# luigifcruz/radio-core

Measured on AMD Instinct MI355X. Metric: IQ Msamples/s through Tuner+WBFM at 1024 channels, higher is better.
Workload: dtype f32

## Files before the change

### include/rcfm_tools.h

```cpp
#ifndef RCFM_TOOLS_H
#define RCFM_TOOLS_H

#include "rcfm.h"

#ifdef __cplusplus
extern "C" {
#endif

typedef struct rcfm_arena_s* rcfm_arena_t;

int rcfm_arena_create(size_t block_bytes, rcfm_arena_t* out);
int rcfm_arena_adopt(void* base, size_t bytes, rcfm_arena_t* out);
int rcfm_arena_bind(rcfm_arena_t arena);
int rcfm_arena_stats(rcfm_arena_t arena, size_t* reserved_bytes, size_t* used_bytes, size_t* live_pieces);
int rcfm_arena_destroy(rcfm_arena_t arena);


enum { RCFM_TUNER_OPT_NARROW_TILES = 1,
       RCFM_TUNER_OPT_ALIGNED_PLAN = 2 };
int rcfm_tuner_set_option(rcfm_tuner_t t, int option, int value);
int rcfm_tuner_load_route(rcfm_tuner_t t, int format, int* route);

enum { RCFM_OPT_LDS_CHAIN = 1, RCFM_OPT_FUSED_TILES = 2, RCFM_OPT_PHASE_LINK = 3, RCFM_OPT_PILOT_CHAIN = 6, RCFM_OPT_DECIM_TILE = 7,
       RCFM_OPT_LDS_DEEMPH = 8, RCFM_OPT_PILOT_BLOCKED = 9, RCFM_OPT_SSB_DIRECT = 11 };
int rcfm_demod_get_option(rcfm_demod_t d, int option, int* value);


typedef struct rcfm_fft_pass {
    int32_t L, nstages, radix[8];
    int64_t n_o1, n_o2, n_inner;
    int64_t in_o1, in_o2, in_i, in_l;
    int64_t out_o1, out_o2, out_i, out_k;
    int64_t tw_o1, tw_o2, tw_i;
    int32_t has_twiddle, load_along_l;
    int64_t in_t, out_t;
    int32_t flat_outer;
    int32_t reserved_;
} rcfm_fft_pass;
typedef struct rcfm_fft_plan {
// ... 29 lines not shown
```

### radio-core_amd/csrc/demod.hip

```cpp

#include <cmath>
#include <cstring>

#include "agc.h"
#include "api_internal.h"

using namespace rcfm;

struct rcfm_demod_s {
    Arena* arena = arena_enter_handle();
    ~rcfm_demod_s() {
        drop_graphs();
        if (cap_stream) (void)hipStreamDestroy(cap_stream);
        arena_leave_handle(arena);
    }
    int kind = 0, C = 0, B = 0, A = 0, ch = 1, chunk = 1;
    double tau = 75e-6;
    float taps_h[51];
    float zi_h[50];
    float pilot_h[41];
    float pilot_g_h[41];
    DeviceBuffer taps, pilot_g;
    struct StateBuf : DeviceBuffer {
        hipEvent_t ev = nullptr;
// ... 18 lines not shown
    float* state_at(int first) const { return state_ptr() + (size_t)first * state_stride(); }
    float side_tap = 0.23f;
    ResampleGeom geom;
    PlanCache r2c_B, c2c_inv_B, c2c_fwd_B, c2c_inv_A, c2r_A;
    std::unique_ptr<FftEngine> eng_B, eng_A;
    std::unique_ptr<FftEngine> eng_Ad;
    std::unique_ptr<FftEngine> eng_Bi;
    DeviceBuffer buf_Ti;
    bool opt_lds_chain = true;
    bool opt_pilot_chain = true;
    bool opt_decim_tile = true;
    bool opt_pilot_blocked = true;
    bool opt_phase_link = true;
    bool opt_lds_deemph = true;
    bool opt_ssb_direct = true;
    int opt_narrow = kNarrowDefault;
    bool opt_graph = false;
    struct GraphSlot {
        const void* iq;
        void* audio;
        const float* state;
        int first;
        hipGraphExec_t exec;
        uint64_t used;
    };
    std::vector<GraphSlot> graphs;
    GraphSlot last_call{nullptr, nullptr, nullptr, -1, nullptr, 0};
    hipStream_t cap_stream = nullptr;
    uint64_t graph_tick = 0;
    void drop_graphs() {
        for (auto& g : graphs) (void)hipGraphExecDestroy(g.exec);
        graphs.clear();
        last_call = GraphSlot{nullptr, nullptr, nullptr, -1, nullptr, 0};
    }
    bool narrow(int cnt) const { return eng_B && narrow_launch(*eng_B, cnt, opt_narrow); }
    DeviceBuffer work, buf_iq, buf_m, buf_p, buf_P, buf_Z, buf_V, buf_v, partial, buf_T, buf_TA, buf_U2, buf_dc;
    int tiles = 0;

    bool decim_plan(const FftEngine& eb, int64_t fa[2]) const {
        const int64_t n1 = eb.desc().pass[0].L;
        fa[0] = A / n1;
        fa[1] = n1;
        FftPlanDesc pa;
        return A % (2 * n1) == 0 && A / n1 >= 16 && fft_plan_describe(A, &pa, 0, fa, 2);
    }

    bool stateful() const { return kind == RCFM_MFM || kind == RCFM_WBFM; }
    bool ssb() const { return kind == RCFM_USB || kind == RCFM_LSB; }

    bool agc_on = false;
    double agc_decay = 0.0;
// ... 68 lines not shown
            if (eng_B->desc().npass == 2 && A < B && decim_plan(*eng_B, fa)) {
                eng_Ad = std::make_unique<FftEngine>(A, fa, 2);
                buf_TA.reserve(c * eng_Ad->tmp_stride() * sizeof(float2));
                if (const int pitch = audio_pitch())
                    buf_V.reserve(c * (size_t)(A / eng_Ad->row_length()) * pitch * sizeof(float2));
            }
            if (kind != RCFM_WBFM) {
                buf_Z.reset(c * B * sizeof(float2));
                buf_V.reset(c * A * sizeof(float2));
            }
        }
        if (kind == RCFM_WBFM) {
            const size_t per_channel = std::max<size_t>((size_t)B, (size_t)pilot_blocked().stride);
            buf_m.reset(c * per_channel * sizeof(float));
            buf_p.reset(c * per_channel * sizeof(float));
        }
    }

    void reset_state(hipStream_t s) {
        if (agc_on) {
            const std::vector<float> all((size_t)C, -1.f);
            RC_HIP(hipMemcpyAsync(state_ptr(), all.data(), all.size() * sizeof(float), hipMemcpyHostToDevice, s));
            RC_HIP(hipStreamSynchronize(s));
        }
        if (!stateful()) return;
        std::vector<float> all((size_t)C * ch * 50);
        for (size_t i = 0; i < all.size(); ++i) all[i] = zi_h[i % 50];
        RC_HIP(hipMemcpyAsync(state_ptr(), all.data(), all.size() * sizeof(float), hipMemcpyHostToDevice, s));
        RC_HIP(hipStreamSynchronize(s));
    }
// ... 222 lines not shown
                TILE_CALL(nw, fused_pilot_chain_mask_mix, *eng_B, *eng_Bi, p, m, T, buf_Ti.as<float2>(), cnt, s, blk.stride,
                          blk.blk16());
            }
            paired = true;
        } else {
            {
                StageTimer tm(ST_FFT_REAL_B, s);
                TILE_CALL(nw, fused_real_pair_fft, *eng_B, p, U2, T, cnt, packed ? kKeepLowerHalf : -1, s);
            }
            if (eng_Bi && opt_pilot_chain) {
                StageTimer tm(ST_IFFT_B, s);
                paired = !packed ? TILE_CALL(nw, fused_hilbert_pair_ifft_mix_fft, *eng_Bi, *eng_B, U2, m, buf_Ti.as<float2>(), T, cnt, s)
                                 : TILE_CALL(nw, fused_hilbert_packed_ifft_mix_fft, *eng_Bi, *eng_B, U2, p, m,
                                             buf_Ti.as<float2>(), T, cnt, s);
            }
        }
        if (paired && eng_Ad && opt_decim_tile && TILE_CALL(nw, fused_fft_decim_ifft_applies, *eng_B, *eng_Ad, cnt)) {
            const int pitch = audio_pitch();
            {
                StageTimer tm(ST_FFT_B, s);
                TILE_CALL(nw, fused_fft_decim_ifft, *eng_B, *eng_Ad, T, V, TA, cnt, geom.wr.as<float>(), geom.scale,
                          buf_dc.as<float2>(), s, pitch);
            }
            run_deemph(reinterpret_cast<float*>(V), audio, first, cnt, s, false, pitch ? (int)eng_Ad->row_length() : 0, pitch);
            return;
        }
        if (paired) {
            StageTimer tm(ST_FFT_B, s);
            TILE_CALL(nw, fused_fft_last_pruned, *eng_B, T, Z, cnt, std::min(A, B) / 2, s);
        } else {
// ... 300 lines not shown

int rcfm_demod_set_option(rcfm_demod_t d, int option, int value) {
    return guarded([&] {
        RC_REQUIRE(d, RCFM_ERR_ARG, "NULL handle");
        d->drop_graphs();
        switch (option) {
            case RCFM_OPT_GRAPH: d->opt_graph = value != 0; break;
            case RCFM_OPT_LDS_CHAIN: d->opt_lds_chain = value != 0; break;
            case RCFM_OPT_FUSED_TILES: d->opt_pilot_chain = d->opt_decim_tile = value != 0; break;
            case RCFM_OPT_PILOT_CHAIN: d->opt_pilot_chain = value != 0; break;
            case RCFM_OPT_DECIM_TILE: d->opt_decim_tile = value != 0; break;
            case RCFM_OPT_PILOT_BLOCKED: d->opt_pilot_blocked = value != 0; break;
            case RCFM_OPT_LDS_DEEMPH: d->opt_lds_deemph = value != 0; break;
            case RCFM_OPT_PHASE_LINK: d->opt_phase_link = value != 0; break;
            case RCFM_OPT_SSB_DIRECT: d->opt_ssb_direct = value != 0; break;
            case RCFM_OPT_NARROW_TILES:
                RC_REQUIRE(value >= 0 && value <= 2, RCFM_ERR_ARG, "narrow tiles: 0 never, 1 automatic, 2 always");
                d->opt_narrow = value;
                break;
            case RCFM_OPT_STATE_FENCE: {
                auto& b = *d->state_buf;
                if (value != 0 && b.ev == nullptr) RC_HIP(hipEventCreateWithFlags(&b.ev, hipEventDisableTiming));
                b.armed = value != 0;
                if (!b.armed) b.recorded = false;
                break;
            }
            default: RC_REQUIRE(false, RCFM_ERR_ARG, "unknown demodulator option");
        }
    });
}
// ... 1 lines not shown
int rcfm_demod_get_option(rcfm_demod_t d, int option, int* value) {
    return guarded([&] {
        RC_REQUIRE(d && value, RCFM_ERR_ARG, "NULL handle or output");
        switch (option) {
            case RCFM_OPT_LDS_CHAIN: *value = d->opt_lds_chain; break;
            case RCFM_OPT_FUSED_TILES: *value = d->opt_pilot_chain && d->opt_decim_tile; break;
            case RCFM_OPT_PILOT_CHAIN: *value = d->opt_pilot_chain; break;
            case RCFM_OPT_DECIM_TILE: *value = d->opt_decim_tile; break;
            case RCFM_OPT_PILOT_BLOCKED:
                *value = d->opt_pilot_blocked && d->opt_pilot_chain && d->pilot_blocked().valid() &&
                         fused_pilot_chain_applies(*d->eng_B, *d->eng_Bi, 2);
                break;
            case RCFM_OPT_LDS_DEEMPH: *value = d->opt_lds_deemph; break;
            case RCFM_OPT_PHASE_LINK: *value = d->opt_phase_link; break;
            case RCFM_OPT_SSB_DIRECT: *value = d->opt_ssb_direct; break;
            case RCFM_OPT_NARROW_TILES: *value = d->opt_narrow; break;
            case RCFM_OPT_STATE_FENCE: *value = d->state_buf->armed; break;
            case RCFM_OPT_GRAPH: *value = d->opt_graph ? 1 + (int)d->graphs.size() : 0; break;
            default: RC_REQUIRE(false, RCFM_ERR_ARG, "unknown demodulator option");
        }
    });
}

int rcfm_demod_set_agc(rcfm_demod_t d, double decay_samples, float level, float floor) {
    return guarded([&] {
        RC_REQUIRE(d, RCFM_ERR_ARG, "NULL handle");
        RC_REQUIRE(d->kind == RCFM_AM || d->ssb(), RCFM_ERR_ARG, "AGC is for AM, USB and LSB demodulators");
        RC_REQUIRE(std::isfinite(decay_samples) && decay_samples >= 0.0, RCFM_ERR_ARG, "AGC decay_samples must be finite and >= 0");
        if (decay_samples == 0.0) {
            d->agc_on = false;
// ... 104 lines not shown
```

### radio-core_amd/csrc/fft_kernel.h

```cpp
#pragma once

#include <hip/hip_runtime.h>

#include <cstdio>
#include <cstdlib>
#include <type_traits>

#include "fft_engine.h"
#include "tile_ns.h"

namespace rcfm {
RCFM_NS_OPEN
namespace fftk {

constexpr int W = RCFM_TILE_W;
constexpr int kLogW = W == 16 ? 4 : W == 8 ? 3 : 2;
static_assert((1 << kLogW) == W, "tile width: 4, 8 or 16 lines");
constexpr int kThreads = 256 * W / 16;

__device__ __forceinline__ float2 cmul(float2 a, float2 b) {
    typedef float v2f __attribute__((ext_vector_type(2)));
    v2f A, B, D;
    A.x = a.x; A.y = a.y; B.x = b.x; B.y = b.y;
    asm("v_pk_mul_f32 %0, %1, %2 op_sel:[0,0] op_sel_hi:[0,1]" : "=v"(D) : "v"(A), "v"(B));
// ... 262 lines not shown
        return load.post(id, l, load.fetch(id, l, base, off), load.prepare(id));
    else
        return load.post(id, l, load.fetch(id, l, base, off));
}

template <class T, class = void>
struct has_half_zones : std::false_type {};
template <class T>
struct has_half_zones<T, std::void_t<decltype(T::kHalfZones)>> : std::bool_constant<T::kHalfZones> {};

template <class T, class = void>
struct has_aux : std::false_type {};
template <class T>
struct has_aux<T, std::void_t<decltype(T::kAux)>> : std::true_type {};

template <class StoreOp>
__device__ __forceinline__ void store_now(const StoreOp& store, const LineId& id, int k, int64_t base, unsigned off,
                                          float2 v) {
    if constexpr (has_aux<StoreOp>::value) store(id, k, base, off, v, store.fetch_aux(id, k, base, off));
    else store(id, k, base, off, v);
}

template <class LoadOp, class StoreOp>
__global__ __launch_bounds__(kThreads) void k_fft_pass(FftPassDev d, LoadOp load, StoreOp store) {
    extern __shared__ __attribute__((aligned(16))) unsigned char smem_raw[];
    const FftPass& p = d.p;
    const int L = p.L;
    float2* tile = reinterpret_cast<float2*>(smem_raw);
    float2* tw = tile + L * W;
    uint16_t* pos = reinterpret_cast<uint16_t*>(tw + L);

    const int tid = threadIdx.x;
    const int64_t tiles_inner = (p.n_inner + W - 1) / W;
    int64_t t = blockIdx.x;
// ... 345 lines not shown
    if constexpr (AUX) {
        const int wc = w < wvalid ? w : 0;
        id.i = i0 + wc;
#pragma unroll
        for (int it = 0; it < nitL; ++it) {
            int g = rg + RG * it;
            if (rowsL % RG != 0) g = g < rowsL ? g : 0;
            const int kb = kbase(g);
#pragma unroll
            for (int q = 0; q < RL; ++q) {
                const int k = kb + (L / RL) * q;
                aux[it * RL + q] = store.fetch_aux(id, k, out_base, (unsigned)k * out_k + (unsigned)wc);
            }
        }
    }

    if constexpr (ROWS) {
#pragma unroll
        for (int it = 0; it < nld; ++it) {
            const int e = tid + T * it;
            const int wl = e / L, l = e - wl * L;
            id.i = i0 + wl;
            float2 x;
            if constexpr (NF == 2) x = load.post(id, l, v[it], v2[it]);
            else x = load.post(id, l, v[it]);
            if ((L * W) % T == 0 || e < L * W) tile[lds_slot<true, !BIG>(l, wl)] = x;
        }
        __syncthreads();
        stage_lds<L, R0, L, true, RG, !BIG, BIG>(tile, tw, w, rg);
    } else {
// ... 57 lines not shown
            for (int q = 0; q < RL; ++q) x[q] = tile[lds_slot<ROWS, !BIG>(g * RL + q, w)];
            dft_p<RL>(x);
            const int kb = kbase(g);
            float2 Tw = make_float2(1.f, 0.f);
            if constexpr (PTW) Tw = big_twiddle(d, f * (unsigned)kb);
            if (lane_ok) {
#pragma unroll
                for (int q = 0; q < RL; ++q) {
                    const int k = kb + (L / RL) * q;
                    float2 y = x[dft_slot<RL>(q)];
                    if constexpr (PTW) {
                        y = cmul(y, Tw);
                        Tw = cmul(Tw, D);
                    }
                    if constexpr (AUX) store(id, k, out_base, (unsigned)k * out_k + (unsigned)w, y, aux[it * RL + q]);
                    else store(id, k, out_base, (unsigned)k * out_k + (unsigned)w, y);
                }
            }
        }
    }
}

template <class T, class = void>
struct mid_upper_rows_zero : std::false_type {};
template <class T>
struct mid_upper_rows_zero<T, std::void_t<decltype(T::kUpperRowsZero)>> : std::bool_constant<T::kUpperRowsZero> {};

template <int L, int R0, int R1, int R2, int R3, int T, class LoadOp, class MidOp, class StoreOp>
__global__ __launch_bounds__(T, (T * 16 / W >= 512 ? 4 : 1)) void k_fft_tile2(FftPassDev d1, FftPassDev d2, LoadOp load,
                                                                     MidOp mid, StoreOp store) {
// ... 560 lines not shown
                    win.dc_bin(id, x);
                }
                tile[lds_slot<true>(l, wl)] = make_float2(x.y, x.x);
            }
        }
        lds_barrier();

        stage_lds<L2, Q0, L2, true, RG>(tile, tw, w, rg);
        lds_barrier();
    }
    if constexpr (S2 == 3) {
        stage_lds<L2, Q1, L2 / Q0, true, RG>(tile, tw, w, rg);
        lds_barrier();
    }
    id.i = i0 + w;
    if (rg < rows2) {
        float2 x[QL];
#pragma unroll
        for (int q = 0; q < QL; ++q) x[q] = tile[lds_slot<true>(rg * QL + q, w)];
        dft_p<QL>(x);
        const float2 D = big_twiddle(d2, f * (unsigned)rows2, seedD);
        float2 Tw = big_twiddle(d2, f * (unsigned)kb2, seedT);
        if (w < wvalid) {
#pragma unroll
            for (int q = 0; q < QL; ++q) {
                const int k = kb2 + rows2 * q;
                const float2 y = cmul(x[dft_slot<QL>(q)], Tw);
                Tw = cmul(Tw, D);
                store(id, k, out_base, (unsigned)k * out_k + (unsigned)w, y);
            }
// ... 236 lines not shown
#define RCFM_CASE(LEN, A, B, C, D, LEN2, E, F, G) fast = fast || (d1.p.L == LEN && d2.p.L == LEN2);
    RCFM_FFT_DECIM_PAIRS(RCFM_CASE)
#undef RCFM_CASE
    return fast && d1.p.load_along_l && !d2.p.load_along_l &&
           d1.p.n_inner == d2.p.n_inner && d1.p.n_o1 * d1.p.n_o2 == 1 && d2.p.n_o1 * d2.p.n_o2 == 1 &&
           d1.p.out_k == d2.p.in_l && d2.p.in_i == 1 && d2.p.out_i == 1 && d2.p.has_twiddle && batch <= 65535;
}

template <class LoadOp, class WinOp, class StoreOp>
inline bool launch_fft_tile2_decim(const FftPassDev& d1, const FftPassDev& d2, int batch, const LoadOp& ld,
                                   const WinOp& win, const StoreOp& st, hipStream_t s) {
    if (!fft_tile2_decim_applies(d1, d2, batch)) return false;
    const dim3 grid((unsigned)((d1.p.n_inner + W - 1) / W), 1, (unsigned)batch);
    bool done = false;
#define RCFM_CASE(LEN, A, B, C, D, LEN2, E, F, G)                                                                \
    if (!done && d1.p.L == LEN && d2.p.L == LEN2) {                                                             \
        hipLaunchKernelGGL((k_fft_tile2_decim<LEN, A, B, C, D, LEN2, E, F, G, tile_threads(LEN), LoadOp, WinOp, StoreOp>), \
                           grid, dim3(tile_threads(LEN)), 0, s, d1, d2, ld, win, st);                           \
        done = true;                                                                                            \
    }
    RCFM_FFT_DECIM_PAIRS(RCFM_CASE)
#undef RCFM_CASE
    if (!done) return false;
    RC_HIP(hipGetLastError());
    return true;
}

template <class LoadOp, class MidOp, class StoreOp>
inline bool launch_fft_tile2_pair(const FftPassDev& d1, const FftPassDev& d2, int count, const LoadOp& ld,
                                  const MidOp& mid, const StoreOp& st, hipStream_t s) {
    const int pairs = (count + 1) / 2;
    if (!fft_tile2_applies(d1, d2, pairs)) return false;
    const dim3 grid((unsigned)((d1.p.n_inner + W - 1) / W), 1, (unsigned)pairs);
    switch (d1.p.L) {
// ... 36 lines not shown
```

### radio-core_amd/csrc/fused_passes.hip

```cpp
#include "fused_passes.h"
#include "device_math.h"

#include "fft_kernel.h"
#include "fft_decim_rt.h"
#include "kernels.h"

namespace rcfm {
RCFM_NS_OPEN

using fftk::LineId;
using fftk::kAnyPass;
using fftk::kRowsOnly;
using fftk::kStridedOnly;

namespace {


struct LoadTunerGatherFast {
    const float2* X;
    const int32_t* base;
    float two_pi_over_n, delta;
    float c0, c1, c2, c3;
    int B, nyq;
    int merge;
// ... 686 lines not shown
        const FftPassDev d1 = ef.pass_dev(1, ef.tmp_stride(), B), d2 = ea.pass_dev(0, A, ea.tmp_stride());
        RC_REQUIRE(fftk::launch_fft_tile2_decim(d1, d2, count, ld, win, st, s) || decim_rt(d1, d2, count, tmp_f, win, tmp_a, s),
                   RCFM_ERR_RUNTIME, "decimating two-transform kernel refused a pair it should accept");
    }
    fftk::LoadPlainT<false> ldl{tmp_a};
    fftk::StorePlainT<true> stl{out, 1.0f};
    FftPassDev last = ea.pass_dev(1, ea.tmp_stride(), A);
    if (out_pitch > 0) {
        RC_REQUIRE(out_pitch >= last.p.out_k && last.p.n_o1 * last.p.n_o2 == 1, RCFM_ERR_RUNTIME, "bad audio row pitch");
        last.out_batch = (A / last.p.out_k) * (int64_t)out_pitch;
        last.p.out_k = out_pitch;
    }
    fftk::launch_fft_pass<kRowsOnly>(last, count, ldl, stl, s);
}

struct StoreRealImagSplit {
    float* y;
    int n, count;
    __device__ __forceinline__ void operator()(const LineId& id, int, int64_t base, unsigned off, float2 v) const {
        const int64_t t = base + off - (int64_t)id.batch * n;
        const int c0 = 2 * id.batch;
        y[(int64_t)c0 * n + t] = v.y;
        if (c0 + 1 < count) y[(int64_t)(c0 + 1) * n + t] = v.x;
    }
};

void fused_real_pair_fft_first(const FftEngine& e, const float* x, float2* tmp, int count, bool from_phase,
                               hipStream_t s, PhaseRows rows) {
    if (count <= 0) return;
    const int64_t n = e.desc().n;
// ... 166 lines not shown
```

### radio-core_amd/csrc/fused_passes_decl.h

```cpp

namespace rcfm {
RCFM_DECL_NS_OPEN


void fused_tuner_ifft(const FftEngine& e, const TunerGather& g, float2* out, float2* tmp, int count,
                      hipStream_t s, float* theta = nullptr, int theta_pitch = 0, bool envelope = false);


void fused_real_fft(const FftEngine& e, const float* x, float2* U, float2* tmp, int count, int keep,
                    hipStream_t s);

void fused_hilbert_ifft(const FftEngine& e, const float2* U, float2* z, float2* tmp, int count, hipStream_t s);

void fused_real_pair_fft(const FftEngine& e, const float* x, float2* U2, float2* tmp, int count, int keep,
                         hipStream_t s, bool from_phase = false, PhaseRows rows = PhaseRows{});
void fused_hilbert_pair_ifft_mix(const FftEngine& e, const float2* U2, const float* m, float2* u, float2* tmp,
                                 int count, hipStream_t s);

bool fused_hilbert_pair_ifft_mix_fft(const FftEngine& ei, const FftEngine& ef, const float2* U2, const float* m,
                                     float2* tmp_i, float2* tmp_f, int count, hipStream_t s);
bool fused_hilbert_packed_applies(const FftEngine& ei, const FftEngine& ef, int count);
bool fused_hilbert_packed_ifft_mix_fft(const FftEngine& ei, const FftEngine& ef, const float2* U2, const float* p,
                                       const float* m, float2* tmp_i, float2* tmp_f, int count, hipStream_t s);
bool fused_pilot_chain_applies(const FftEngine& ef, const FftEngine& ei, int count);
bool fused_pilot_chain_geometry(const FftEngine& ef, int64_t* rows, int64_t* row_length);
void fused_pilot_chain_fft_first(const FftEngine& ef, const float* p, float2* tmp_f, int count, hipStream_t s,
                                 int64_t blk_stride = 0, int blk16 = 0);
void fused_pilot_chain_mask_mix(const FftEngine& ef, const FftEngine& ei, const float* p, const float* m,
                                float2* tmp_f, float2* tmp_i, int count, hipStream_t s, int64_t blk_stride = 0,
                                int blk16 = 0);

void fused_fft_last_pruned(const FftEngine& ef, const float2* tmp_f, float2* out, int count, int keep,
                           hipStream_t s);

bool fused_fft_decim_ifft_applies(const FftEngine& ef, const FftEngine& ea, int count);
void fused_fft_decim_ifft(const FftEngine& ef, const FftEngine& ea, const float2* tmp_f, float2* out, float2* tmp_a,
                          int count, const float* wr, float scale, float2* dc, hipStream_t s, int out_pitch = 0);

void fused_real_pair_fft_first(const FftEngine& e, const float* x, float2* tmp, int count, bool from_phase,
                               hipStream_t s, PhaseRows rows = PhaseRows{});
void fused_fft_decim_ifft_pairs(const FftEngine& ef, const FftEngine& ea, const float2* tmp_f, float* y,
                                float2* tmp_a, int count, const float* wr, float scale, float2* dc, hipStream_t s);

void fused_stereo_unpack_ifft(const FftEngine& e, const float2* U, int64_t B, float2* out, float2* tmp, int count,
                              const float* wr, int nyq, int nmin, float nyq_factor, float scale, float2* dc,
                              hipStream_t s);

void fused_fft_pruned(const FftEngine& e, const float2* in, float2* out, float2* tmp, int count, int keep,
                      hipStream_t s);

void fused_ifft_real_out(const FftEngine& e, const float2* Y, float* y, float2* tmp, int count, float scale,
                         hipStream_t s);

// ... 6 lines not shown
```

### radio-core_amd/csrc/kernels.h

```cpp
#pragma once

#include "common.h"

namespace rcfm {

enum NyquistMode : int { NYQ_NONE = 0, NYQ_DOWN = 1, NYQ_UP = 2 };

void launch_spectrum_c2c(const float2* X, int64_t x_stride, int64_t n, const int64_t* roll, float2* Y,
                         int64_t m, int batch, const float* wpos, const float* wneg, float w_merge,
                         int nyq, int nneg, int nyq_mode, float scale, hipStream_t stream);

void launch_spectrum_r2c(const float2* X, int64_t n, float2* Y, int64_t m, int batch, const float* wr,
                         int nyq, int nmin, float nyq_factor, float scale, hipStream_t stream);

void launch_spectrum_real_full(const float2* X, int64_t n, float2* Y, int64_t m, int batch, const float* wr,
                               int nyq, int nmin, float nyq_factor, float scale, float2* dc, bool paired,
                               hipStream_t stream);

void launch_hilbert_mask(const float2* P, float2* Z, int64_t n, int batch, float scale,
                         hipStream_t stream);

void launch_stereo_unpack(const float2* U, int64_t B, float2* V, int64_t A, int batch, const float* wr,
                          int nyq, int nmin, float nyq_factor, float scale, float2* dc, hipStream_t stream);

// ... 25 lines not shown

constexpr int kMaxBatch = 65535;
constexpr int kFirMaxTaps = 5461;
constexpr int kPilotMaxTaps = 2867;

int fir_tiles(int64_t n);
void launch_fir(const float* x, float* y, int64_t n, int ch, int batch, const float* taps, int nb,
                const float* state, float* partial, hipStream_t stream);
int fir51_tiles(int64_t n, int ch);
void launch_fir51(const float* x, float* y, int64_t n, int ch, int batch, const float* taps_host,
                  const float* state, float* partial, const float2* dc, hipStream_t stream, int row_samples = 0,
                  int row_pitch_samples = 0);
void launch_fir_state(const float* x, int64_t n, int ch, int batch, const float* taps, int nb,
                      float* state, hipStream_t stream, int row_samples = 0,
                      int row_pitch_samples = 0);
void launch_dc_clip(float* y, int64_t n, int ch, int batch, const float* partial, int nparts,
                    hipStream_t stream);

void launch_envelope(const float2* iq, float* e, int64_t n, hipStream_t stream);
void launch_am_tail(float* y, int64_t n, int batch, const float2* dc, hipStream_t stream);

void launch_ssb_select(const float2* X, int64_t n, float2* Y, int64_t m, int batch, const float* wr, int kmax,
                       int nyq_bin, float nyq_factor, float scale, bool lower, hipStream_t stream);
void launch_ssb_tail(float* y, int64_t n, int batch, float level, hipStream_t stream);

int level_segments(int64_t B);
void launch_channel_levels(const float2* X, int64_t N, const int32_t* base, const int64_t* roll, const int32_t* bw,
                           int count, int max_segments, double* part, float* power, hipStream_t stream);
struct CarrierPart {
    double s0, s1, s2, mx;
// ... 15 lines not shown
```

### radio-core_amd/csrc/kernels.hip

```cpp

#include "kernels.h"

#include <climits>
#include <cmath>
#include "device_math.h"

namespace rcfm {

namespace {

constexpr int kThreads = 256;
constexpr float kInvPi = 0.31830988618379067154f;

__device__ __forceinline__ float2 cscale(float2 a, float s) { return make_float2(a.x * s, a.y * s); }

inline dim3 grid2(int64_t items, int per_block, int batch) {
    return dim3((unsigned)((items + per_block - 1) / per_block), (unsigned)batch, 1);
}


__global__ __launch_bounds__(kThreads) void k_spectrum_c2c(
    const float2* __restrict__ X, int64_t x_stride, int64_t n, const int64_t* __restrict__ roll,
    float2* __restrict__ Y, int64_t m, const float* __restrict__ wpos, const float* __restrict__ wneg,
    float w_merge, int nyq, int nneg, int nyq_mode, float scale) {
// ... 680 lines not shown
    const int h = blockIdx.x % ch, c = blockIdx.x / ch;
    const float* xc = x + (int64_t)c * lay.signal_stride;
    float* zc = state + ((int64_t)c * ch + h) * (nb - 1);
    for (int s = threadIdx.x; s < nb - 1; s += blockDim.x) {
        z_old[s] = zc[s];
        xt[s] = (s < n) ? xc[lay.at((n - 1 - s) * ch + h)] : 0.f;
    }
    for (int s = threadIdx.x; s < nb; s += blockDim.x) tp[s] = taps[s];
    __syncthreads();
    for (int s = threadIdx.x; s < nb - 1; s += blockDim.x) {
        float acc = 0.f;
        const int cnt = (int)((nb - 1 - s) < n ? (nb - 1 - s) : n);
        for (int i = 0; i < cnt; ++i) acc = fmaf(tp[s + 1 + i], xt[i], acc);
        if (s + n < nb - 1) acc += z_old[s + n];
        zc[s] = acc;
    }
}

__global__ __launch_bounds__(kThreads) void k_dc_clip(float* __restrict__ y, int64_t total,
                                                      const float* __restrict__ partial, int nparts) {
    __shared__ float mean_s;
    const int c = blockIdx.y;
    if (threadIdx.x < 64) {
        double acc = 0.0;
        for (int i = threadIdx.x; i < nparts; i += 64) acc += (double)partial[(int64_t)c * nparts + i];
        for (int off = 32; off > 0; off >>= 1) acc += __shfl_down(acc, off, 64);
        if (threadIdx.x == 0) mean_s = (float)(acc / (double)total);
    }
    __syncthreads();
    const float mean = mean_s;
// ... 689 lines not shown
    if (ch == 2)
        hipLaunchKernelGGL(k_fir51<2>, grid, dim3(kThreads), 0, stream, x, y, n * 2, taps, state, partial, dc, lay);
    else
        hipLaunchKernelGGL(k_fir51<1>, grid, dim3(kThreads), 0, stream, x, y, n, taps, state, partial, dc, lay);
    RC_LAUNCH_CHECK();
}

void launch_fir_state(const float* x, int64_t n, int ch, int batch, const float* taps, int nb,
                      float* state, hipStream_t stream, int row_samples, int row_pitch_samples) {
    if (batch <= 0 || nb < 2) return;
    hipLaunchKernelGGL(k_fir_state, dim3((unsigned)(batch * ch)), dim3(128), fir_state_lds_bytes(nb), stream,
                       x, n, ch, taps, nb, state, row_layout(n, ch, row_samples, row_pitch_samples));
    RC_LAUNCH_CHECK();
}

void launch_dc_clip(float* y, int64_t n, int ch, int batch, const float* partial, int nparts,
                    hipStream_t stream) {
    if (batch <= 0) return;
    const int64_t total = n * ch;
    hipLaunchKernelGGL(k_dc_clip, grid2(total, kThreads, batch), dim3(kThreads), 0, stream, y, total, partial,
                       nparts);
    RC_LAUNCH_CHECK();
}

void launch_envelope(const float2* iq, float* e, int64_t n, hipStream_t stream) {
    if (n <= 0) return;
    if (((uintptr_t)iq | (uintptr_t)e) % 16 == 0)
        hipLaunchKernelGGL(k_envelope<true>, grid2((n + 3) / 4, kThreads, 1), dim3(kThreads), 0, stream, iq, e, n);
    else
        hipLaunchKernelGGL(k_envelope<false>, grid2(n, kThreads, 1), dim3(kThreads), 0, stream, iq, e, n);
// ... 128 lines not shown
```

### radio-core_amd/radiocore/_internal/hip.py

```python

import ctypes
import os
import sys
import threading
import warnings

import numpy as np

_HERE = os.path.dirname(os.path.abspath(__file__))
LIB_PATH = os.environ.get("RCFM_LIB") or os.path.join(os.path.dirname(_HERE), "_lib", "librcfm.so")

RCFM_FM, RCFM_MFM, RCFM_WBFM = 0, 1, 2
RCFM_AM = 3
RCFM_USB, RCFM_LSB = 5, 6
RCFM_SSB_LEVEL = 0.25
RCFM_AGC_PEAK, RCFM_AGC_CARRIER = 0, 1
RCFM_OPT_LDS_CHAIN, RCFM_OPT_FUSED_TILES, RCFM_OPT_PHASE_LINK, RCFM_OPT_NARROW_TILES, RCFM_OPT_STATE_FENCE = 1, 2, 3, 4, 5
RCFM_OPT_PILOT_CHAIN, RCFM_OPT_DECIM_TILE, RCFM_OPT_LDS_DEEMPH, RCFM_OPT_PILOT_BLOCKED, RCFM_OPT_GRAPH = 6, 7, 8, 9, 10
RCFM_OPT_SSB_DIRECT = 11
RCFM_IQ_CS16, RCFM_IQ_CS8, RCFM_IQ_CU8 = 1, 2, 3
RCFM_IQ_CF32 = 0
RCFM_BLANK_MEDIAN, RCFM_BLANK_ABSOLUTE = 0, 1
RCFM_BLANK_MIN_BLOCK, RCFM_BLANK_MAX_BLOCK, RCFM_BLANK_MAX_SPAN, RCFM_BLANK_MAX_GUARD = 64, 1 << 20, 8, 1024
RCFM_PCM_F32, RCFM_PCM_S16 = 0, 1
RCFM_PACK_SEGMENT = 4096
RCFM_IQ_BALANCE_OFF, RCFM_IQ_BALANCE_FIXED, RCFM_IQ_BALANCE_AUTO = 0, 1, 2
RCFM_IQ_SEG_PAIRS, RCFM_IQ_MAX_SEGS = 16384, 1024
RCFM_TONE_MAX_K, RCFM_TONE_SEGMENT = 64, 8192
RCFM_SOS_MAX_SECTIONS, RCFM_SOS_RUN, RCFM_SOS_SEGMENT = 8, 33, 8192
RCFM_GATE_WAVE_FLOATS, RCFM_GATE_SEG_FLOATS, RCFM_GATE_MAX_FRAMES, RCFM_GATE_MAX_RAMP = 4096, 16384, 65535, 1 << 20
RCFM_FLOOR_MAX_HALF, RCFM_FLOOR_MAX_CELLS = 4096, 1 << 30
RCFM_TUNER_OPT_NARROW_TILES,RCFM_TUNER_OPT_ALIGNED_PLAN = 1, 2

_ERR_SIZE, _ERR_INDEX, _ERR_RUNTIME, _ERR_ARG, _ERR_STATE = -1, -2, -3, -4, -5
# ... 351 lines not shown
```

Baseline: 35190.

## Fuse de-emphasis FIR into decimating FFT tile with tail-state finish kernel

Adds a new WBFM path that applies the 51-tap de-emphasis FIR in the frequency-domain tile of the decimating FFT pair. It writes per-tile tail partials, reduces them in a small finish kernel that updates filter state, a boundary correction and the mean, and applies correction, DC removal and clipping in the final inverse-FFT store. This replaces the separate de-emphasis FIR, state and DC/clip kernels and their extra passes over audio memory. In exchange it adds three launches, extra tail buffers, LDS pressure in the tile kernel and a recursive FIR formulation that depends on the taps being geometric.

```diff
diff --git a/include/rcfm_tools.h b/include/rcfm_tools.h
--- a/include/rcfm_tools.h
+++ b/include/rcfm_tools.h
@@ -22,7 +22,7 @@
 int rcfm_tuner_load_route(rcfm_tuner_t t, int format, int* route);
 
 enum { RCFM_OPT_LDS_CHAIN = 1, RCFM_OPT_FUSED_TILES = 2, RCFM_OPT_PHASE_LINK = 3, RCFM_OPT_PILOT_CHAIN = 6, RCFM_OPT_DECIM_TILE = 7,
-       RCFM_OPT_LDS_DEEMPH = 8, RCFM_OPT_PILOT_BLOCKED = 9, RCFM_OPT_SSB_DIRECT = 11 };
+       RCFM_OPT_LDS_DEEMPH = 8, RCFM_OPT_PILOT_BLOCKED = 9, RCFM_OPT_SSB_DIRECT = 11, RCFM_OPT_DEEMPH_TILE = 12 };
 int rcfm_demod_get_option(rcfm_demod_t d, int option, int* value);
 
 
diff --git a/radio-core_amd/csrc/demod.hip b/radio-core_amd/csrc/demod.hip
--- a/radio-core_amd/csrc/demod.hip
+++ b/radio-core_amd/csrc/demod.hip
@@ -6,6 +6,10 @@
 #include "api_internal.h"
 
 using namespace rcfm;
+
+#ifndef RCFM_DEEMPH_TILE_DEFAULT
+#define RCFM_DEEMPH_TILE_DEFAULT 1
+#endif
 
 struct rcfm_demod_s {
     Arena* arena = arena_enter_handle();
@@ -56,6 +60,7 @@
     bool opt_phase_link = true;
     bool opt_lds_deemph = true;
     bool opt_ssb_direct = true;
+    bool opt_deemph_tile = RCFM_DEEMPH_TILE_DEFAULT;
     int opt_narrow = kNarrowDefault;
     bool opt_graph = false;
     struct GraphSlot {
@@ -77,6 +82,7 @@
     }
     bool narrow(int cnt) const { return eng_B && narrow_launch(*eng_B, cnt, opt_narrow); }
     DeviceBuffer work, buf_iq, buf_m, buf_p, buf_P, buf_Z, buf_V, buf_v, partial, buf_T, buf_TA, buf_U2, buf_dc;
+    DeviceBuffer buf_tail, buf_corr, buf_mean;
     int tiles = 0;
 
     bool decim_plan(const FftEngine& eb, int64_t fa[2]) const {
@@ -175,6 +181,11 @@
             const size_t per_channel = std::max<size_t>((size_t)B, (size_t)pilot_blocked().stride);
             buf_m.reset(c * per_channel * sizeof(float));
             buf_p.reset(c * per_channel * sizeof(float));
+            if (eng_B && eng_Ad && deemph_fused() && fused_fft_decim_deemph_applies(*eng_B, *eng_Ad, 1)) {
+                buf_tail.reset(c * (size_t)fused_deemph_tile_count(*eng_Ad) * 50 * sizeof(float2));
+                buf_corr.reset(c * 50 * sizeof(float2));
+                buf_mean.reset(c * sizeof(float));
+            }
         }
     }
 
@@ -427,6 +438,25 @@
                                  : TILE_CALL(nw, fused_hilbert_packed_ifft_mix_fft, *eng_Bi, *eng_B, U2, p, m,
                                              buf_Ti.as<float2>(), T, cnt, s);
             }
+        }
+        if (paired && eng_Ad && opt_decim_tile && opt_deemph_tile && buf_tail.bytes() != 0 && deemph_geometric() &&
+            TILE_CALL(nw, fused_fft_decim_deemph_applies, *eng_B, *eng_Ad, cnt)) {
+            {
+                StageTimer tm(ST_FFT_B, s);
+                TILE_CALL(nw, fused_fft_decim_deemph_tile, *eng_B, *eng_Ad, T, TA, cnt, geom.wr.as<float>(), geom.scale,
+                          buf_dc.as<float2>(), taps_h, buf_tail.as<float2>(), s);
+            }
+            {
+                StateFence fence(*this, s);
+                StageTimer tm(ST_DEEMPH, s);
+                launch_deemph_finish(buf_tail.as<float2>(), fused_deemph_tile_count(*eng_Ad),
+                                     (int)((eng_Ad->desc().pass[0].n_inner + 7) / 8), A, cnt, taps_h,
+                                     buf_dc.as<float2>(), state_at(first), buf_corr.as<float2>(), buf_mean.as<float>(), s);
+            }
+            StageTimer tm(ST_FFT_B, s);
+            TILE_CALL(nw, fused_ifft_last_deemph, *eng_Ad, TA, reinterpret_cast<float2*>(audio), cnt, buf_corr.as<float2>(),
+                      buf_mean.as<float>(), s);
+            return;
         }
         if (paired && eng_Ad && opt_decim_tile && TILE_CALL(nw, fused_fft_decim_ifft_applies, *eng_B, *eng_Ad, cnt)) {
             const int pitch = audio_pitch();
@@ -757,6 +787,7 @@
             case RCFM_OPT_LDS_DEEMPH: d->opt_lds_deemph = value != 0; break;
             case RCFM_OPT_PHASE_LINK: d->opt_phase_link = value != 0; break;
             case RCFM_OPT_SSB_DIRECT: d->opt_ssb_direct = value != 0; break;
+            case RCFM_OPT_DEEMPH_TILE: d->opt_deemph_tile = value != 0; break;
             case RCFM_OPT_NARROW_TILES:
                 RC_REQUIRE(value >= 0 && value <= 2, RCFM_ERR_ARG, "narrow tiles: 0 never, 1 automatic, 2 always");
                 d->opt_narrow = value;
@@ -788,6 +819,7 @@
             case RCFM_OPT_LDS_DEEMPH: *value = d->opt_lds_deemph; break;
             case RCFM_OPT_PHASE_LINK: *value = d->opt_phase_link; break;
             case RCFM_OPT_SSB_DIRECT: *value = d->opt_ssb_direct; break;
+            case RCFM_OPT_DEEMPH_TILE: *value = d->opt_deemph_tile; break;
             case RCFM_OPT_NARROW_TILES: *value = d->opt_narrow; break;
             case RCFM_OPT_STATE_FENCE: *value = d->state_buf->armed; break;
             case RCFM_OPT_GRAPH: *value = d->opt_graph ? 1 + (int)d->graphs.size() : 0; break;
diff --git a/radio-core_amd/csrc/fft_kernel.h b/radio-core_amd/csrc/fft_kernel.h
--- a/radio-core_amd/csrc/fft_kernel.h
+++ b/radio-core_amd/csrc/fft_kernel.h
@@ -300,10 +300,28 @@
 template <class T>
 struct has_aux<T, std::void_t<decltype(T::kAux)>> : std::true_type {};
 
+template <class T, class = void>
+struct has_store_ctx : std::false_type {};
+template <class T>
+struct has_store_ctx<T, std::void_t<decltype(T::kStoreCtx)>> : std::true_type {};
+
+template <class T, class = void>
+struct has_deemph_tile : std::false_type {};
+template <class T>
+struct has_deemph_tile<T, std::void_t<decltype(T::kDeemphTile)>> : std::true_type {};
+
+struct FirTaps51 {
+    float b[51];
+};
+constexpr int kDeemphHist = 50;
+constexpr int deemph_tail_groups(int n_inner) { return 2 * ((n_inner + 15) / 16); }
+constexpr bool deemph_tile_fits(int L, int L2) { return L2 > kDeemphHist && L2 + kDeemphHist + 1 <= L; }
+
 template <class StoreOp>
 __device__ __forceinline__ void store_now(const StoreOp& store, const LineId& id, int k, int64_t base, unsigned off,
                                           float2 v) {
     if constexpr (has_aux<StoreOp>::value) store(id, k, base, off, v, store.fetch_aux(id, k, base, off));
+    else if constexpr (has_store_ctx<StoreOp>::value) store(id, k, base, off, v, store.prepare(id));
     else store(id, k, base, off, v);
 }
 
@@ -679,6 +697,17 @@
             }
         }
     }
+    constexpr bool SCTX = has_store_ctx<StoreOp>::value;
+    static_assert(!SCTX || (ROWS && !AUX), "store context: rows passes without auxiliary inputs only");
+    auto sctx = [&] {
+        if constexpr (SCTX) {
+            LineId li = id;
+            li.i = i0 + (w < wvalid ? w : 0);
+            return store.prepare(li);
+        } else {
+            return 0;
+        }
+    }();
 
     if constexpr (ROWS) {
 #pragma unroll
@@ -766,6 +795,7 @@
                         Tw = cmul(Tw, D);
                     }
                     if constexpr (AUX) store(id, k, out_base, (unsigned)k * out_k + (unsigned)w, y, aux[it * RL + q]);
+                    else if constexpr (SCTX) store(id, k, out_base, (unsigned)k * out_k + (unsigned)w, y, sctx);
                     else store(id, k, out_base, (unsigned)k * out_k + (unsigned)w, y);
                 }
             }
@@ -1356,6 +1386,78 @@
         lds_barrier();
     }
     id.i = i0 + w;
+    if constexpr (has_deemph_tile<StoreOp>::value) {
+        static_assert(L2 > kDeemphHist, "one borrow from the slow time digit at most");
+        static_assert(RG > rows2, "the tail partials run on the butterfly rows the last stage leaves idle");
+        static_assert(L2 + kDeemphHist + 1 <= L, "Z_1 and its 51 borrowed columns fit the tile's image");
+        float2 phi;
+        sincospif(2.0f * ((float)(i0 + w) / (float)p2.n_inner), &phi.y, &phi.x);
+        float2 x[QL];
+        if (rg < rows2) {
+#pragma unroll
+            for (int q = 0; q < QL; ++q) x[q] = tile[lds_slot<true>(rg * QL + q, w)];
+            dft_p<QL>(x);
+        }
+        lds_barrier();
+        constexpr int H1 = kDeemphHist + 1;
+        if (rg < rows2) {
+            const float2 D = big_twiddle(d2, f * (unsigned)rows2, seedD);
+            float2 Tw = big_twiddle(d2, f * (unsigned)kb2, seedT);
+#pragma unroll
+            for (int q = 0; q < QL; ++q) {
+                const int k = kb2 + rows2 * q;
+                const float2 v = cmul(x[dft_slot<QL>(q)], Tw);
+                Tw = cmul(Tw, D);
+                tile[lds_slot<true>(k + H1, w)] = v;
+                if (rows2 * q >= L2 - H1 || (rows2 * (q + 1) > L2 - H1 && k >= L2 - H1))
+                    tile[lds_slot<true>(k - (L2 - H1), w)] = cmul(v, phi);
+            }
+        }
+        lds_barrier();
+        if (rg < rows2) {
+            const FirTaps51& tp = store.taps;
+            const int e0 = rg * QL;
+            const float2* zp = &tile[lds_slot<true>(e0, w)];
+            float2 y[QL];
+            float2 ap[4];
+#pragma unroll
+            for (int i = 0; i < 4; ++i) ap[i] = make_float2(0.f, 0.f);
+#pragma unroll
+            for (int j = 1; j <= kDeemphHist; ++j) {
+                const float2 z = zp[(H1 - j) * kRowsPitch];
+                ap[j & 3].x = fmaf(tp.b[j], z.x, ap[j & 3].x);
+                ap[j & 3].y = fmaf(tp.b[j], z.y, ap[j & 3].y);
+            }
+            y[0] = make_float2((ap[0].x + ap[1].x) + (ap[2].x + ap[3].x), (ap[0].y + ap[1].y) + (ap[2].y + ap[3].y));
+            const float xr = tp.b[2] / tp.b[1];
+            const float tl = xr * tp.b[kDeemphHist];
+#pragma unroll
+            for (int r = 1; r < QL; ++r) {
+                const float2 zn = zp[(r + kDeemphHist) * kRowsPitch], zo = zp[r * kRowsPitch];
+                y[r].x = fmaf(xr, y[r - 1].x, fmaf(tp.b[1], zn.x, -tl * zo.x));
+                y[r].y = fmaf(xr, y[r - 1].y, fmaf(tp.b[1], zn.y, -tl * zo.y));
+            }
+            if (w < wvalid) {
+#pragma unroll
+                for (int r = 0; r < QL; ++r)
+                    store(id, e0 + r, out_base, (unsigned)(e0 + r) * out_k + (unsigned)w, y[r]);
+            }
+        } else {
+            const int ngrp = deemph_tail_groups((int)p1.n_inner);
+            float2* tail = store.tail + ((int64_t)id.batch * ngrp + ((i0 + w) >> 3)) * kDeemphHist;
+            for (int t = rg - rows2; t < kDeemphHist; t += RG - rows2) {
+                float2 v = tile[lds_slot<true>(t + 1, w)];
+                if (w >= wvalid) v = make_float2(0.f, 0.f);
+#pragma unroll
+                for (int off = 4; off > 0; off >>= 1) {
+                    v.x += __shfl_xor(v.x, off, 8);
+                    v.y += __shfl_xor(v.y, off, 8);
+                }
+                if ((w & 7) == 0) tail[t] = v;
+            }
+        }
+        return;
+    }
     if (rg < rows2) {
         float2 x[QL];
 #pragma unroll
@@ -1622,10 +1724,12 @@
     const dim3 grid((unsigned)((d1.p.n_inner + W - 1) / W), 1, (unsigned)batch);
     bool done = false;
 #define RCFM_CASE(LEN, A, B, C, D, LEN2, E, F, G)                                                                \
-    if (!done && d1.p.L == LEN && d2.p.L == LEN2) {                                                             \
-        hipLaunchKernelGGL((k_fft_tile2_decim<LEN, A, B, C, D, LEN2, E, F, G, tile_threads(LEN), LoadOp, WinOp, StoreOp>), \
-                           grid, dim3(tile_threads(LEN)), 0, s, d1, d2, ld, win, st);                           \
-        done = true;                                                                                            \
+    if constexpr (!has_deemph_tile<StoreOp>::value || deemph_tile_fits(LEN, LEN2)) {                            \
+        if (!done && d1.p.L == LEN && d2.p.L == LEN2) {                                                         \
+            hipLaunchKernelGGL((k_fft_tile2_decim<LEN, A, B, C, D, LEN2, E, F, G, tile_threads(LEN), LoadOp, WinOp, StoreOp>), \
+                               grid, dim3(tile_threads(LEN)), 0, s, d1, d2, ld, win, st);                       \
+            done = true;                                                                                        \
+        }                                                                                                       \
     }
     RCFM_FFT_DECIM_PAIRS(RCFM_CASE)
 #undef RCFM_CASE
diff --git a/radio-core_amd/csrc/fused_passes.hip b/radio-core_amd/csrc/fused_passes.hip
--- a/radio-core_amd/csrc/fused_passes.hip
+++ b/radio-core_amd/csrc/fused_passes.hip
@@ -724,6 +724,89 @@
     fftk::launch_fft_pass<kRowsOnly>(last, count, ldl, stl, s);
 }
 
+struct StoreDeemphTile {
+    static constexpr bool kDeemphTile = true;
+    float2* out;
+    float2* tail;
+    fftk::FirTaps51 taps;
+    __device__ __forceinline__ void operator()(const LineId&, int, int64_t base, unsigned off, float2 v) const {
+        fftk::stream_store(out + base + off, v);
+    }
+};
+
+#ifndef RCFM_DEEMPH_AUDIO_NT
+#define RCFM_DEEMPH_AUDIO_NT 0
+#endif
+struct StoreAudioDeemph {
+    static __device__ __forceinline__ void audio_store(float2* p, float2 v) {
+        if constexpr (RCFM_DEEMPH_AUDIO_NT) fftk::stream_store(p, v);
+        else *p = v;
+    }
+    static constexpr bool kStoreCtx = true;
+    float2* out;
+    const float2* corr;
+    const float* mean;
+    struct Ctx {
+        float2 corr;
+        float mean;
+    };
+    __device__ __forceinline__ Ctx prepare(const LineId& id) const {
+        Ctx c;
+        c.mean = mean[id.batch];
+        c.corr = id.i < fftk::kDeemphHist ? corr[(int64_t)id.batch * fftk::kDeemphHist + id.i] : make_float2(0.f, 0.f);
+        return c;
+    }
+    __device__ __forceinline__ void operator()(const LineId&, int k, int64_t base, unsigned off, float2 v,
+                                               const Ctx& c) const {
+        float l = v.y, r = v.x;
+        if (k == 0) {
+            l += c.corr.x;
+            r += c.corr.y;
+        }
+        l -= c.mean;
+        r -= c.mean;
+        l = (l < -0.999f) ? -0.999f : ((l > 0.999f) ? 0.999f : l);
+        r = (r < -0.999f) ? -0.999f : ((r > 0.999f) ? 0.999f : r);
+        audio_store(out + base + off, make_float2(l, r));
+    }
+};
+
+bool fused_fft_decim_deemph_applies(const FftEngine& ef, const FftEngine& ea, int count) {
+    if (ef.npass() != 2 || ea.npass() != 2) return false;
+    const int64_t B = ef.desc().n, A = ea.desc().n;
+    if (A >= B || (A & 1) || ea.desc().pass[1].L != ef.desc().pass[0].L) return false;
+    const FftPassDev d1 = ef.pass_dev(1, ef.tmp_stride(), B), d2 = ea.pass_dev(0, A, ea.tmp_stride());
+    const FftPass& last = ea.desc().pass[1];
+    return fftk::fft_tile2_decim_applies(d1, d2, count) && fftk::deemph_tile_fits(d1.p.L, d2.p.L) && last.n_o1 * last.n_o2 == 1 &&
+           last.n_inner == d2.p.L;
+}
+
+int fused_deemph_tile_count(const FftEngine& ea) {
+    return fftk::deemph_tail_groups((int)ea.desc().pass[0].n_inner);
+}
+
+void fused_fft_decim_deemph_tile(const FftEngine& ef, const FftEngine& ea, const float2* tmp_f, float2* tmp_a, int count,
+                                 const float* wr, float scale, float2* dc, const float* taps_host, float2* tail,
+                                 hipStream_t s) {
+    if (count <= 0) return;
+    const int64_t B = ef.desc().n, A = ea.desc().n;
+    fftk::LoadPlainT<false> ld{tmp_f};
+    WinAudioDecim win{wr, dc, scale, (int)A, ef.desc().pass[0].L, 0};
+    StoreDeemphTile st{tmp_a, tail, {}};
+    for (int i = 0; i < 51; ++i) st.taps.b[i] = taps_host[i];
+    const FftPassDev d1 = ef.pass_dev(1, ef.tmp_stride(), B), d2 = ea.pass_dev(0, A, ea.tmp_stride());
+    RC_REQUIRE(fftk::launch_fft_tile2_decim(d1, d2, count, ld, win, st, s), RCFM_ERR_RUNTIME,
+               "decimating two-transform kernel refused a pair it should accept");
+}
+
+void fused_ifft_last_deemph(const FftEngine& ea, const float2* tmp_a, float2* out, int count, const float2* corr,
+                            const float* mean, hipStream_t s) {
+    if (count <= 0) return;
+    fftk::LoadPlainT<false> ldl{tmp_a};
+    StoreAudioDeemph stl{out, corr, mean};
+    fftk::launch_fft_pass<kRowsOnly>(ea.pass_dev(1, ea.tmp_stride(), ea.desc().n), count, ldl, stl, s);
+}
+
 struct StoreRealImagSplit {
     float* y;
     int n, count;
diff --git a/radio-core_amd/csrc/fused_passes_decl.h b/radio-core_amd/csrc/fused_passes_decl.h
--- a/radio-core_amd/csrc/fused_passes_decl.h
+++ b/radio-core_amd/csrc/fused_passes_decl.h
@@ -37,6 +37,14 @@
 void fused_fft_decim_ifft(const FftEngine& ef, const FftEngine& ea, const float2* tmp_f, float2* out, float2* tmp_a,
                           int count, const float* wr, float scale, float2* dc, hipStream_t s, int out_pitch = 0);
 
+bool fused_fft_decim_deemph_applies(const FftEngine& ef, const FftEngine& ea, int count);
+int fused_deemph_tile_count(const FftEngine& ea);
+void fused_fft_decim_deemph_tile(const FftEngine& ef, const FftEngine& ea, const float2* tmp_f, float2* tmp_a, int count,
+                                 const float* wr, float scale, float2* dc, const float* taps_host, float2* tail,
+                                 hipStream_t s);
+void fused_ifft_last_deemph(const FftEngine& ea, const float2* tmp_a, float2* out, int count, const float2* corr,
+                            const float* mean, hipStream_t s);
+
 void fused_real_pair_fft_first(const FftEngine& e, const float* x, float2* tmp, int count, bool from_phase,
                                hipStream_t s, PhaseRows rows = PhaseRows{});
 void fused_fft_decim_ifft_pairs(const FftEngine& ef, const FftEngine& ea, const float2* tmp_f, float* y,
diff --git a/radio-core_amd/csrc/kernels.h b/radio-core_amd/csrc/kernels.h
--- a/radio-core_amd/csrc/kernels.h
+++ b/radio-core_amd/csrc/kernels.h
@@ -63,6 +63,8 @@
 void launch_fir_state(const float* x, int64_t n, int ch, int batch, const float* taps, int nb,
                       float* state, hipStream_t stream, int row_samples = 0,
                       int row_pitch_samples = 0);
+void launch_deemph_finish(const float2* partial, int stride, int ngroups, int64_t n, int batch, const float* taps_host,
+                          const float2* dc, float* state, float2* corr, float* mean, hipStream_t stream);
 void launch_dc_clip(float* y, int64_t n, int ch, int batch, const float* partial, int nparts,
                     hipStream_t stream);
 
diff --git a/radio-core_amd/csrc/kernels.hip b/radio-core_amd/csrc/kernels.hip
--- a/radio-core_amd/csrc/kernels.hip
+++ b/radio-core_amd/csrc/kernels.hip
@@ -718,6 +718,52 @@
         for (int i = 0; i < cnt; ++i) acc = fmaf(tp[s + 1 + i], xt[i], acc);
         if (s + n < nb - 1) acc += z_old[s + n];
         zc[s] = acc;
+    }
+}
+
+__global__ __launch_bounds__(128) void k_deemph_finish(const float2* __restrict__ partial, int stride, int ngroups, int64_t A,
+                                                        DeemphTaps taps, const float2* __restrict__ dc,
+                                                        float* __restrict__ state, float2* __restrict__ corr,
+                                                        float* __restrict__ mean) {
+    __shared__ float xt[2][50];
+    __shared__ float red[2];
+    const int c = blockIdx.x, tid = threadIdx.x;
+    const int h = tid >= 64, s = tid & 63;
+    if (tid < 50) {
+        const float2* p = partial + (int64_t)c * stride * 50 + tid;
+        float2 acc = make_float2(0.f, 0.f);
+#pragma unroll 6
+        for (int t = 0; t < ngroups; ++t) {
+            acc.x += p[(int64_t)t * 50].x;
+            acc.y += p[(int64_t)t * 50].y;
+        }
+        xt[0][49 - tid] = acc.y;
+        xt[1][49 - tid] = acc.x;
+    }
+    __syncthreads();
+    float d = 0.f;
+    if (s < 50) {
+        float* zc = state + ((int64_t)c * 2 + h) * 50;
+        float acc = 0.f;
+#pragma unroll
+        for (int i = 0; i < 50; ++i) {
+            const float b = taps.b[i + 1];
+            const int k = i - s;
+            acc = fmaf(b, k >= 0 ? xt[h][k] : 0.f, acc);
+        }
+        d = zc[s] - acc;
+        zc[s] = acc;
+        reinterpret_cast<float*>(corr + (int64_t)c * 50 + s)[h] = d;
+    }
+    for (int off = 32; off > 0; off >>= 1) d += __shfl_down(d, off, 64);
+    if (s == 0) red[h] = d;
+    __syncthreads();
+    if (tid == 0) {
+        float bsum = 0.f;
+#pragma unroll
+        for (int j = 0; j <= 50; ++j) bsum += taps.b[j];
+        const float2 d0 = dc[c];
+        mean[c] = ((float)A * (d0.x + d0.y) * bsum + red[0] + red[1]) / (float)(2 * A);
     }
 }
 
@@ -1437,6 +1483,16 @@
     RC_LAUNCH_CHECK();
 }
 
+void launch_deemph_finish(const float2* partial, int stride, int ngroups, int64_t n, int batch, const float* taps_host,
+                          const float2* dc, float* state, float2* corr, float* mean, hipStream_t stream) {
+    if (batch <= 0) return;
+    DeemphTaps taps;
+    for (int i = 0; i < 51; ++i) taps.b[i] = taps_host[i];
+    hipLaunchKernelGGL(k_deemph_finish, dim3((unsigned)batch), dim3(128), 0, stream, partial, stride, ngroups, n, taps, dc, state,
+                       corr, mean);
+    RC_LAUNCH_CHECK();
+}
+
 void launch_dc_clip(float* y, int64_t n, int ch, int batch, const float* partial, int nparts,
                     hipStream_t stream) {
     if (batch <= 0) return;
diff --git a/radio-core_amd/radiocore/_internal/hip.py b/radio-core_amd/radiocore/_internal/hip.py
--- a/radio-core_amd/radiocore/_internal/hip.py
+++ b/radio-core_amd/radiocore/_internal/hip.py
@@ -18,6 +18,7 @@
 RCFM_OPT_LDS_CHAIN, RCFM_OPT_FUSED_TILES, RCFM_OPT_PHASE_LINK, RCFM_OPT_NARROW_TILES, RCFM_OPT_STATE_FENCE = 1, 2, 3, 4, 5
 RCFM_OPT_PILOT_CHAIN, RCFM_OPT_DECIM_TILE, RCFM_OPT_LDS_DEEMPH, RCFM_OPT_PILOT_BLOCKED, RCFM_OPT_GRAPH = 6, 7, 8, 9, 10
 RCFM_OPT_SSB_DIRECT = 11
+RCFM_OPT_DEEMPH_TILE = 12
 RCFM_IQ_CS16, RCFM_IQ_CS8, RCFM_IQ_CU8 = 1, 2, 3
 RCFM_IQ_CF32 = 0
 RCFM_BLANK_MEDIAN, RCFM_BLANK_ABSOLUTE = 0, 1
```

New measurement: 35500, median of 6. No clear change (+0.9%).
